# voutcn/megahit

Hardware: AMD Instinct MI355X
Metric: M (k+1)-mer edges sorted+counted/sec, sdbg_build k=21 (higher is better)
Workload: dtype u32; 1 GPU; read2sdbg (S1+S2) k=21 m=2 no mercy, 10000000 synthetic 150 bp PE reads per GPU (BASELINE configs[1]), inputs resident in HBM, outputs left in HBM; reads_per_gpu=10000000, edges_per_gpu=1290000000, k=21, min_count=2, parallelism=1 GPU, s1_items=1330000000, s2_items=117381042, sdbg_records=59857080

## Files before the change

### megahit_amd/csrc/mhx_internal.h

```cpp
#pragma once
#include <hip/hip_runtime.h>

#include <cstdint>
#include <cstdio>
#include <cstring>
#include <functional>
#include <map>
#include <stdexcept>
#include <string>
#include <vector>

#include "../../include/mhx.h"

namespace mhx {

struct OnesweepLaunch;
void set_error(const char *fmt, ...);

struct Error : std::runtime_error {
  explicit Error(const std::string &s) : std::runtime_error(s) {}
};

#define MHX_HIP(expr)                                                                          \
  do {                                                                                         \
// ... 99 lines not shown
    (ctx)->prof_begin(name, bytes);       \
    __VA_ARGS__;                          \
    MHX_HIP(hipGetLastError());           \
    (ctx)->prof_end();                    \
  } while (0)

namespace mhx {

struct SortPass {
  int shift;
  int bits;
  int shift2 = 0;
  int bits2 = 0;
  int prev_lo = -1;
};
struct SortPrep {
  const void *buf = nullptr;
  uint64_t n = 0;
  int hist_passes = 0;
  uint64_t hist_sig = 0;
  std::function<void(const OnesweepLaunch &)> gen;
  uint64_t gen_slots = 0;
  bool gen_var = false;
};
uint32_t *radix_sort(mhx_ctx *c, uint32_t *buf_a, uint32_t *buf_b, uint64_t n, int stride, int key_words,
                     const std::vector<SortPass> &passes, SortPrep *prep = nullptr);
uint32_t *sort_whole_key(mhx_ctx *c, uint32_t *buf_a, uint32_t *buf_b, uint64_t n, int stride, int key_words,
                         const std::vector<SortPass> &passes, SortPrep *prep = nullptr);
std::vector<SortPass> make_passes(int key_words, int lo_bit, int hi_bit);
bool sort_takes_generated_first_pass(const mhx_ctx *c, uint64_t n, int stride, const std::vector<SortPass> &passes);
uint64_t passes_signature(const std::vector<SortPass> &ps);
uint32_t *kmsort_exact(mhx_ctx *c, uint32_t *buf_a, uint32_t *buf_b, uint64_t n, int S, int key_words, SortPrep *prep = nullptr);

void exclusive_scan_u32_u64(mhx_ctx *c, const uint32_t *in, uint64_t *out, uint64_t n, uint64_t *d_total);
void exclusive_scan_u64(mhx_ctx *c, const uint64_t *in, uint64_t *out, uint64_t n, uint64_t *d_total);
void find_group_heads(mhx_ctx *c, const uint32_t *items, uint64_t n, int stride, int cmp_bits,
                      uint64_t *heads, uint64_t *d_count);
uint64_t count_group_heads(mhx_ctx *c, const uint32_t *items, uint64_t n, int stride, int cmp_bits);

struct DigitSpec;
DigitSpec spec_of_pass(const SortPass &ps, int key_words);
std::vector<SortPass> make_passes_ranges(int key_words, const std::vector<std::pair<int, int>> &ranges);
void emit_sdbg(mhx_ctx *c, const uint32_t *sorted, uint64_t n_items, int S, int kw, uint32_t k, int is_seq, mhx_sdbg_result *out, int compact_bits = 0);

void partition_by_owner(mhx_ctx *c, const uint32_t *a, uint32_t *b, uint64_t n, int stride, const uint8_t *lut, int n_parts,
                        uint64_t *counts);
uint64_t s1_extract(mhx_ctx *c, uint32_t k, bool compact, SortPrep *prep, bool defer_items = false, bool filter_in_gen = false);
bool s1_compact(const mhx_ctx *c, uint32_t k, int want_mercy);
bool s1_rank_tagged(const mhx_ctx *c, uint32_t k);
int s1_stride(uint32_t k, bool compact);
struct S1Sources {
  int n = 0;
  std::vector<const uint32_t *> ptr;
// ... 136 lines not shown
```

### megahit_amd/csrc/s1_skm.hip

```cpp
#include <cstring>

#include "s1_shared.h"

namespace mhx {

constexpr int kSkmC = 8;
constexpr int kSkmW = 10;
constexpr int kSkmNM = kSkmC + kSkmW - 1;
constexpr int kSkmMinBinBits = 16, kSkmMaxBinBits = 20;

__device__ __forceinline__ uint32_t skm_mix(uint32_t c) {
  uint32_t h = c * 0x9E3779B1u;
  return h ^ (h >> 15);
}
__device__ __forceinline__ uint32_t skm_mix2(uint32_t c) {
  uint32_t h = c * 0x9E3779B1u;
  h ^= h >> 15;
  return h * 0x85EBCA6Bu;
}
__device__ __forceinline__ uint32_t skm_bin_of(uint32_t minh) {
  return (minh ^ (minh >> 16)) * 0x7FEB352Du;
}

template <int NT, int J, bool VAR, bool COUNT = false>
__global__ __launch_bounds__(NT) void k_skm_make(const uint32_t *__restrict__ seq, const uint64_t *__restrict__ start, uint32_t L, uint32_t bpr, uint64_t n_blocks,
                                                 int k, int bin_bits, uint32_t bin_lo, uint32_t bin_hi, int count_items, uint64_t pos_base,
                                                 unsigned long long *__restrict__ hp, uint4 *__restrict__ out, unsigned long long cap,
                                                 unsigned long long *__restrict__ cursor, uint32_t *__restrict__ err, unsigned long long *__restrict__ digit_hist) {
  __shared__ uint32_t sm_scan[NT / kWave + 1];
  __shared__ unsigned long long s_base;
  __shared__ uint32_t dh[3][256];
  __shared__ uint32_t lbin[J * kSkmC][NT];
  __shared__ uint32_t hpl[2][12];
  const int tid = threadIdx.x;
  if (tid < 24) hpl[tid / 12][tid % 12] = 0;
  for (int i = tid; i < 768; i += NT) dh[i >> 8][i & 255] = 0;
  __syncthreads();
  const bool third_digit = bin_bits > 16;
  const int M = k + 1 - (kSkmW - 1);
  const uint32_t mmask = (1u << (2 * M)) - 1u;
  const int K1 = k + 1;
  const unsigned bin_sh = 32u - (unsigned)bin_bits;
  unsigned long long items = 0;
  uint32_t hp_n[2] = {0, 0};
  unsigned long long hp_p[2] = {~0ull, ~0ull};
  for (uint64_t it = blockIdx.x; it * (uint64_t)(NT * J) < n_blocks; it += gridDim.x) {
    uint64_t Wv[J], pos0[J];
    uint32_t smask[J], emask[J];
    uint32_t bflag[J];
#pragma unroll
    for (int j = 0; j < J; ++j) {
      const uint64_t b = it * (uint64_t)(NT * J) + (uint64_t)j * NT + tid;
      smask[j] = 0;
      emask[j] = 0;
      bflag[j] = 0;
      Wv[j] = 0;
      pos0[j] = 0;
      if (b < n_blocks) {
        const uint64_t r = b / bpr;
        const uint32_t q0 = (uint32_t)(b - r * bpr) * kSkmC;
        uint64_t base;
        uint32_t nwin;
        if constexpr (VAR) {
          base = start[r];
          const uint64_t len_r = start[r + 1] - base;
          nwin = len_r >= (uint64_t)K1 ? (uint32_t)(len_r - k) : 0u;
          if (q0 == 0 && nwin && count_items) items += nwin + (COUNT ? 0 : 4);
        } else {
          base = r * L;
          nwin = L - k;
        }
        if (q0 < nwin) {
// ... 2 lines not shown
          const unsigned sh = (unsigned)(a & 15) * 2;
          const uint32_t c0 = seq[wi], c1 = seq[wi + 1], c2 = seq[wi + 2];
          const uint64_t W = ((uint64_t)funnel_l(c0, c1, sh) << 32) | funnel_l(c1, c2, sh);
          const uint64_t R = rc64(W, 32);
          uint32_t h[kSkmNM];
#pragma unroll
          for (int i = 0; i < kSkmNM; ++i) {
            const uint32_t f = (uint32_t)(W >> (64 - 2 * (i + M))) & mmask;
            const uint32_t rv = (uint32_t)(R >> (2 * i)) & mmask;
            h[i] = skm_mix(min(f, rv));
          }
          uint32_t sfx[kSkmW];
          sfx[kSkmW - 1] = h[kSkmW - 1];
#pragma unroll
          for (int i = kSkmW - 2; i >= 0; --i) sfx[i] = min(h[i], sfx[i + 1]);
          uint32_t pfx = 0xFFFFFFFFu;
          uint32_t bins[kSkmC];
          bins[0] = skm_bin_of(sfx[0]) >> bin_sh;
#pragma unroll
          for (int w = 1; w < kSkmC; ++w) {
            pfx = min(pfx, h[kSkmW - 1 + w]);
            bins[w] = skm_bin_of(min(sfx[w], pfx)) >> bin_sh;
          }
#pragma unroll
          for (int w = 0; w < kSkmC; ++w) lbin[j * kSkmC + w][tid] = bins[w];
          const uint32_t n_here = min((uint32_t)kSkmC, nwin - q0);
          uint32_t km = 0, sm = 0, hm = 0;
          if (hp) {
            const uint64_t dx = W ^ (W << 2);
#pragma unroll
            for (int w = 0; w < kSkmC; ++w)
              if ((uint32_t)w < n_here && ((dx << (2 * w)) >> (64 - 2 * (K1 - 1))) == 0) hm |= 1u << w;
            if (hm && count_items) {
#pragma unroll
              for (int w = 0; w < kSkmC; ++w)
                if ((hm >> w) & 1u) {
                  const unsigned b = (unsigned)(W >> (62 - 2 * w)) & 3u;
                  const unsigned cls = b == 0 || b == 3 ? 0u : 1u;
                  if constexpr (COUNT) {
                    const bool strand = b >= 2;
                    const unsigned prev_raw = q0 + w == 0 ? kSentinel
                                              : (w == 0 ? (unsigned)((seq[(a - 1) >> 4] >> (30 - 2 * (unsigned)((a - 1) & 15))) & 3u) : (unsigned)(W >> (64 - 2 * w)) & 3u);
                    const unsigned next_raw = q0 + w + 1 == nwin ? kSentinel : (unsigned)(W >> (62 - 2 * (w + K1))) & 3u;
                    const unsigned pv = strand ? comp_or_sentinel(next_raw) : prev_raw, nx = strand ? comp_or_sentinel(prev_raw) : next_raw;
                    atomicAdd(&hpl[cls][0], 1u);
                    if (pv < 4) atomicAdd(&hpl[cls][1 + pv], 1u);
                    if (nx < 4) atomicAdd(&hpl[cls][5 + nx], 1u);
                  } else {
// ... 2 lines not shown
                  }
                }
            }
          }
#pragma unroll
          for (int w = 0; w < kSkmC; ++w)
            if ((uint32_t)w < n_here && !((hm >> w) & 1u) && bins[w] >= bin_lo && bins[w] < bin_hi) km |= 1u << w;
#pragma unroll
          for (int w = 0; w < kSkmC; ++w)
            if (((km >> w) & 1u) && (w == 0 || !((km >> (w - 1)) & 1u) || bins[w] != bins[w > 0 ? w - 1 : 0])) sm |= 1u << w;
          smask[j] = sm;
          emask[j] = km & ((sm >> 1) | ~(km >> 1));
          if constexpr (COUNT) {
            const uint64_t pb = a > 0 ? (uint64_t)((seq[(a - 1) >> 4] >> (30 - 2 * (unsigned)((a - 1) & 15))) & 3u) : 0ull;
            Wv[j] = (W >> 2) | (pb << 62);
            bflag[j] = (q0 == 0 ? 1u : 0u) | (q0 + n_here == nwin ? 2u : 0u) | (n_here << 2);
          } else {
            Wv[j] = W;
          }
          pos0[j] = pos_base + a;
        }
      }
    }
    uint32_t cnt = 0;
#pragma unroll
    for (int j = 0; j < J; ++j) cnt += (uint32_t)__builtin_popcount(smask[j]);
    uint32_t total = 0;
    const uint32_t excl = block_exclusive_sum<uint32_t, NT>(cnt, sm_scan, &total);
    if (tid == 0) s_base = total ? atomicAdd(cursor, (unsigned long long)total) : 0ull;
    __syncthreads();
    const unsigned long long base = s_base;
    if (base + total > cap) {
      if (tid == 0) atomicOr(err, 1u);
      return;
    }
    unsigned long long at = base + excl;
#pragma unroll
    for (int j = 0; j < J; ++j) {
      uint32_t sm = smask[j], em = emask[j];
      while (sm) {
        const int rs = __builtin_ctz(sm), re = __builtin_ctz(em);
        sm &= sm - 1;
        em &= em - 1;
        const int len = re - rs + 1;
        const uint32_t run_bin = lbin[j * kSkmC + rs][tid];
        const uint64_t p = pos0[j] + (uint64_t)rs;
        if constexpr (COUNT) {
          const uint64_t bases = (Wv[j] << (2 * rs)) & (~0ull << (64 - 2 * (K1 + len + 1)));
          const uint32_t n_blk = bflag[j] >> 2;
          const uint32_t fl = ((bflag[j] & 1u) && rs == 0 ? 16u : 0u) | ((bflag[j] & 2u) && (uint32_t)(re + 1) == n_blk ? 8u : 0u);
          out[at++] = make_uint4((run_bin << 8) | ((uint32_t)(p >> 32) << 28) | ((uint32_t)(len - 1) << 5) | fl, (uint32_t)(bases >> 32), (uint32_t)bases, (uint32_t)p);
        } else {
        const uint64_t bases = ((Wv[j] << (2 * rs)) & (~0ull << (64 - 2 * (K1 + len - 1)))) | (uint64_t)(len - 1);
        out[at++] = make_uint4((run_bin << 8) | ((uint32_t)(p >> 32) << 28), (uint32_t)(bases >> 32), (uint32_t)bases, (uint32_t)p);
        }
        atomicAdd(&dh[0][run_bin & 255u], 1u);
        atomicAdd(&dh[1][(run_bin >> 8) & 255u], 1u);
        if (third_digit) atomicAdd(&dh[2][run_bin >> 16], 1u);
      }
    }
  }
  if constexpr (VAR) {
    items = wave_sum(items);
    if ((tid & (kWave - 1)) == 0 && items) atomicAdd(cursor + 3, items);
  }
  if constexpr (COUNT) {
    __syncthreads();
    if (hp && count_items && tid < 24 && hpl[tid / 12][tid % 12]) atomicAdd(hp + 8 + (tid / 12) * 16 + (tid % 12), (unsigned long long)hpl[tid / 12][tid % 12]);
  }
  if (!COUNT && hp && count_items) {
#pragma unroll
    for (int x = 0; x < 2; ++x) {
      const uint32_t n_w = wave_sum(hp_n[x]);
      if (n_w) {
        unsigned long long pmin = hp_p[x];
#pragma unroll
        for (int d = kWave / 2; d > 0; d >>= 1) pmin = min(pmin, (unsigned long long)__shfl_xor((long long)pmin, d, kWave));
        if ((tid & (kWave - 1)) == 0) {
          atomicAdd(hp + x, (unsigned long long)n_w);
          atomicMin(hp + 2 + x, pmin);
        }
      }
    }
// ... 30 lines not shown
}

__global__ __launch_bounds__(256) void k_skm_bounds(const uint4 *__restrict__ recs, uint64_t n, uint32_t n_bins, uint64_t *__restrict__ bounds,
                                                    uint32_t *__restrict__ max_bin) {
  const uint32_t b = blockIdx.x * 256 + threadIdx.x;
  if (b > n_bins) return;
  auto lower = [&](uint32_t v) -> uint64_t {
    uint64_t lo = 0, hi = n;
    while (lo < hi) {
      const uint64_t mid = (lo + hi) >> 1;
      const uint32_t bin = (reinterpret_cast<const uint32_t *>(recs + mid)[0] >> 8) & 0xFFFFFu;
      if (bin < v) lo = mid + 1;
      else hi = mid;
    }
    return lo;
  };
  const uint64_t at = b == n_bins ? n : lower(b);
  bounds[b] = at;
  if (b < n_bins) {
    const uint64_t nx = b + 1 == n_bins ? n : lower(b + 1);
    const uint64_t d = nx - at;
    atomicMax(max_bin, d > 0xFFFFFFFFull ? 0xFFFFFFFFu : (uint32_t)d);
  }
}

struct SkmArgs {
  int k;
  uint32_t m;
  uint8_t *solid_bytes;
  unsigned long long *hist;
  uint2 *agg_raw;
  uint32_t agg_cap;
  uint32_t *agg_counts;
  uint32_t *err;
  uint32_t max_fill;
  int probe_limit;
  uint32_t bin_lo, bin_hi;
  unsigned long long *marks_raw;
  uint32_t marks_cap;
  uint32_t *marks_counts;
};
struct SkmSrcs {
  const uint4 *ptr[kSkmSrcMax];
  const uint64_t *bounds[kSkmSrcMax];
  int n;
};
// ... 862 lines not shown
  const double need = (double)n_win * (double)std::max<long long>(c->opt("s1_skm_cap_pct", 36), 1) / 100.0 * 32.0;
  const double budget = (double)std::max<long long>(c->opt("s1_skm_pass_gb", 48), 1) * 1e9;
  return (int)std::min(64.0, std::max(1.0, std::ceil(need / budget)));
}

bool s1_skm_front(mhx_ctx *c, uint32_t k, SkmFront *f, int pass, int n_passes, int bin_bits_agreed, bool for_count) {
  SeqSet &s = c->seqs;
  hipStream_t st = c->stream;
  const bool var = s.fixed_len == 0;
  const uint32_t L = var ? s.max_len : s.fixed_len, bpr = (L - k + kSkmC - 1) / kSkmC;
  const uint64_t n_blocks = s.n_seqs * (uint64_t)bpr;
  const uint64_t n_win = var ? (s.n_bases > s.n_seqs * (uint64_t)k ? s.n_bases - s.n_seqs * (uint64_t)k : 0) : s.n_seqs * (uint64_t)(L - k);
  const uint64_t cap_all = n_win * (uint64_t)std::max<long long>(c->opt("s1_skm_cap_pct", 36), 1) / 100;
  const uint64_t cap = std::max<uint64_t>(n_passes > 1 ? cap_all / n_passes + cap_all / n_passes * 15 / 100 : cap_all, 1u << 16);
  int bin_bits = kSkmMinBinBits;
  while (bin_bits < kSkmMaxBinBits && (double)n_win * 0.29 / (double)(1ull << bin_bits) > 8192.0) ++bin_bits;
  if (const long long fb = c->opt("s1_skm_bin_bits", 0)) bin_bits = (int)std::min<long long>(kSkmMaxBinBits, std::max<long long>(8, fb));
  if (bin_bits_agreed > 0) bin_bits = bin_bits_agreed;
  uint4 *buf_a = c->ws("items_a", cap * 16 + 64).as<uint4>();
  uint4 *buf_b = c->ws("items_b", cap * 16 + 64).as<uint4>();
  unsigned long long *cursor = c->ws("skm_cursor", 64).as<unsigned long long>();
  uint32_t *err = reinterpret_cast<uint32_t *>(cursor + 1);
  uint32_t *max_bin = err + 1;
  MHX_HIP(hipMemsetAsync(cursor, 0, 64, st));
  std::vector<SortPass> passes;
  for (int lo = 0; lo < bin_bits; lo += 8) passes.push_back(SortPass{8 + lo, std::min(8, bin_bits - lo), 0, 0, 0});
  unsigned long long *pre_hist = c->ws("sort_pre_hist", (size_t)kMaxFusedPasses * 256 * 8).as<unsigned long long>();
  MHX_HIP(hipMemsetAsync(pre_hist, 0, (size_t)3 * 256 * 8, st));
  constexpr int NT = 512, J = 2;
  const uint64_t cus = c->n_cus > 0 ? (uint64_t)c->n_cus : 256;
  const unsigned grid = (unsigned)std::min<uint64_t>(div_ceil(n_blocks, (uint64_t)NT * J), cus * 8);
  const uint32_t n_bins = 1u << bin_bits;
  const uint32_t bin_lo = (uint32_t)((uint64_t)n_bins * pass / n_passes), bin_hi = (uint32_t)((uint64_t)n_bins * (pass + 1) / n_passes);
  unsigned long long *hp = nullptr;
  if (!c->global_bases && c->opt("s1_skm_hp", 1)) {
    hp = c->ws("skm_hp", 512).as<unsigned long long>();
    if (pass == 0) {
      unsigned long long init[48] = {0};
      init[2] = init[3] = ~0ull;
      MHX_HIP(hipMemcpyAsync(hp, init, sizeof init, hipMemcpyHostToDevice, st));
      MHX_HIP(hipStreamSynchronize(st));
    }
  }
#define MHX_MAKE(VARV, COUNTV)                                                                                                                                   \
  hipLaunchKernelGGL((k_skm_make<NT, J, VARV, COUNTV>), dim3(grid), dim3(NT), 0, st, s.words.as<uint32_t>(), s.start.as<uint64_t>(), L, bpr, n_blocks, (int)k, \
                     bin_bits, bin_lo, bin_hi, pass == 0 ? 1 : 0, c->pos_base, hp, buf_a, (unsigned long long)cap, cursor, err, pre_hist)
  MHX_LAUNCH(c, for_count ? "count_skm_make" : "s1_skm_make", (double)s.n_bases / 4 + (double)n_win * 16 / 3.5, {
    if (var && for_count) MHX_MAKE(true, true);
    else if (var) MHX_MAKE(true, false);
    else if (for_count) MHX_MAKE(false, true);
    else MHX_MAKE(false, false);
  });
#undef MHX_MAKE
  unsigned long long h[4] = {0, 0, 0, 0};
  std::vector<unsigned long long> h_dh(passes.size() * 256);
  MHX_HIP(hipMemcpyAsync(h, cursor, 32, hipMemcpyDeviceToHost, st));
  MHX_HIP(hipMemcpyAsync(h_dh.data(), pre_hist, h_dh.size() * 8, hipMemcpyDeviceToHost, st));
  MHX_HIP(hipStreamSynchronize(st));
  f->n_records = 0;
  f->hp = hp;
  if ((uint32_t)h[1] != 0 || h[0] > cap) return false;
  const uint64_t n = h[0];
  {
    const uint64_t n_bins_pass = std::max<uint64_t>(1, ((1ull << bin_bits) + n_passes - 1) / n_passes);
    const uint64_t limit = std::max<uint64_t>((uint64_t)c->opt("s1_skm_max_bin", 1 << 16), 16 * (n / n_bins_pass + 1));
    bool all = n > 0;
    uint64_t smallest_excess = ~0ull;
    for (size_t p = 0; p < passes.size() && all; ++p) {
      const uint64_t vals = 1ull << passes[p].bits;
      uint64_t mx = 0;
      for (uint64_t d = 0; d < vals; ++d) mx = std::max<uint64_t>(mx, h_dh[p * 256 + d]);
      const uint64_t mean = n / std::max<uint64_t>(1, (p + 1 == passes.size() && n_passes > 1) ? std::max<uint64_t>(1, vals / n_passes) : vals);
      const uint64_t excess = mx > mean ? mx - mean : 0;
      smallest_excess = std::min(smallest_excess, excess);
      all = excess >= limit + limit / 2;
    }
    if (all) {
      f->n_records = n;
      f->max_bin = (uint32_t)std::min<uint64_t>(smallest_excess, 0xFFFFFFFFu);
      return false;
    }
  }
  SortPrep prep;
  prep.buf = buf_a;
  prep.n = n;
  prep.hist_passes = (int)passes.size();
  prep.hist_sig = passes_signature(passes);
  uint32_t *sorted = radix_sort(c, reinterpret_cast<uint32_t *>(buf_a), reinterpret_cast<uint32_t *>(buf_b), n, 4, 1, passes, &prep);
  uint64_t *bounds = c->ws("s1_bucket_bounds", ((size_t)n_bins + 1) * 8 + 64).as<uint64_t>();
  MHX_LAUNCH(c, "s1_skm_bounds", (double)n_bins * 8 * 30,
             hipLaunchKernelGGL(k_skm_bounds, dim3((n_bins + 1 + 255) / 256), dim3(256), 0, st, reinterpret_cast<const uint4 *>(sorted), n, n_bins, bounds, max_bin));
  uint32_t h_max = 0;
  MHX_HIP(hipMemcpyAsync(&h_max, max_bin, 4, hipMemcpyDeviceToHost, st));
  MHX_HIP(hipStreamSynchronize(st));
  f->n_src = 1;
  f->src[0] = reinterpret_cast<const uint4 *>(sorted);
  f->src_bounds[0] = bounds;
  f->spare = sorted == reinterpret_cast<uint32_t *>(buf_a) ? reinterpret_cast<uint32_t *>(buf_b) : reinterpret_cast<uint32_t *>(buf_a);
  f->spare_bytes = cap * 16;
  f->n_records = n;
  f->n_windows = n_win;
  if (pass == 0) f->n_items = var ? h[3] : s.n_seqs * (uint64_t)(L - k + (for_count ? 0 : 4));
  f->n_bins = n_bins;
  f->bin_lo = bin_lo;
  f->bin_hi = bin_hi;
  f->bin_bits = bin_bits;
  f->max_bin = h_max;
  const uint64_t limit = std::max<uint64_t>((uint64_t)c->opt("s1_skm_max_bin", 1 << 16), 16 * (n / (bin_hi - bin_lo) + 1));
  return h_max <= limit;
}

// ... 125 lines not shown
```

### megahit_amd/csrc/sort.hip

```cpp
#include "dev_prims.h"
#include <cstdlib>
#include <cstring>
#include <string>

#include "mhx_internal.h"
#include "sort_digits.h"
#include "sort_kernels.h"

namespace mhx {

template <int S, int NI>
__global__ __launch_bounds__(kSortThreads) void k_radix_hist(const uint32_t *__restrict__ items, uint64_t n, DigitSpec ds,
                                                             uint32_t *__restrict__ hist, uint64_t n_chunks,
                                                             const uint8_t *__restrict__ lut) {
  __shared__ uint32_t h[kSortWaves][256];
  for (int i = threadIdx.x; i < kSortWaves * 256; i += kSortThreads) (&h[0][0])[i] = 0;
  __syncthreads();
  const int w = threadIdx.x / kWave;
  const uint64_t base = (uint64_t)blockIdx.x * SortCfg<S, NI>::kChunk;
  for (int j = 0; j < SortCfg<S, NI>::kChunk / kSortThreads; ++j) {
    uint64_t idx = base + (uint64_t)j * kSortThreads + threadIdx.x;
    if (idx < n) {
      const uint32_t *p = items + idx * S;
      unsigned d;
// ... 202 lines not shown
    ds.wi2 = key_words - 1 - ps.shift2 / 32;
    ds.bit2 = (unsigned)(ps.shift2 % 32);
    ds.mask2 = (1u << ps.bits2) - 1;
    ds.sh2 = (unsigned)ps.bits;
  }
  if (ps.prev_lo >= 0 && ps.prev_lo < ps.shift && !ps.bits2 && ps.prev_lo / 32 == (ps.shift + ps.bits - 1) / 32) {
    const unsigned hi = (unsigned)(ps.shift % 32), lo = (unsigned)(ps.prev_lo % 32);
    ds.prev_mask = ((1u << hi) - 1u) & ~((1u << lo) - 1u);
  }
  return ds;
}

struct SortEnv {
  bool classic;
  std::string shape;
  int items;
};
static SortEnv sort_env() {
  const char *e = getenv("MHX_SORT"), *sh = getenv("MHX_SORT_SHAPE"), *it = getenv("MHX_SORT_ITEMS");
  return SortEnv{e && !strcmp(e, "classic"), sh ? sh : "", it ? atoi(it) : 0};
}
static void refuse_unconsumed_generator(const SortPrep &prep, const char *who) {
  if (prep.gen) throw Error(std::string(who) + ": the records of this buffer are to be made by a generated first pass, which this sort path cannot run");
}

template <int S, int NI, int UT>
static uint32_t *radix_sort_onesweep(mhx_ctx *c, uint32_t *a, uint32_t *b, uint64_t n, int key_words, const std::vector<SortPass> &passes,
                                     const SortPrep &prep) {
  const int P = (int)passes.size();
  const bool prep_fits = prep.buf == (const void *)a && prep.n == n;
  const bool gen = prep.gen && prep_fits && S == 3 && NI == 8 && UT == 3;
  if (!gen) refuse_unconsumed_generator(prep, "radix sort (chained scan)");
  const uint64_t gen_slots = gen ? std::max<uint64_t>(prep.gen_slots, n) : n;
  const int xcd_units = c->opt("sort_xcd_units", 1) != 0 && c->n_cus >= 192;
  const uint64_t unit = (uint64_t)kSortThreads * NI * UT;
  auto units_of = [&](uint64_t items) { return xcd_units ? (div_ceil(items, unit) + 127) / 128 * 128 : div_ceil(items, unit); };
  const uint64_t n_units = units_of(n), n_units_gen = units_of(gen_slots);
  hipStream_t st = c->stream;
  constexpr bool kCanUt2 = S == 3 && NI == 8 && UT == 3;
  const bool loaded_ut2 = kCanUt2 && c->opt("sort_loaded_ut2", 0) != 0;
  const uint64_t unit2 = (uint64_t)kSortThreads * NI * 2;
  const uint64_t n_units2 = xcd_units ? (div_ceil(n, unit2) + 127) / 128 * 128 : div_ceil(n, unit2);
  const uint64_t n_status = std::max(n_units_gen, loaded_ut2 ? n_units2 : 0);
  unsigned long long *status = c->ws("sort_status", n_status * 256 * 8).as<unsigned long long>();
  unsigned long long *gh = c->ws("sort_ghist", (size_t)2 * kMaxChainedPasses * 256 * 8).as<unsigned long long>();
  unsigned long long *starts = gh + kMaxChainedPasses * 256;
  constexpr int kErrSlot = kMaxChainedPasses * 8;
  uint32_t *tickets = c->ws("sort_tickets", (kErrSlot + 8) * 4).as<uint32_t>();
  MHX_HIP(hipMemsetAsync(status, 0, n_status * 256 * 8, st));
  MHX_HIP(hipMemsetAsync(gh, 0, (size_t)kMaxChainedPasses * 256 * 8, st));
  MHX_HIP(hipMemsetAsync(tickets, 0, (kErrSlot + 8) * 4, st));
  const double bytes = (double)n * S * 4;
  static const std::string nm_hist = "radix_hist_all_" + std::to_string(S * 4) + "B", nm_scat = "radix_scatter_" + std::to_string(S * 4) + "B";
  const unsigned hgrid = (unsigned)std::min<uint64_t>(div_ceil(n, (uint64_t)kSortThreads * 16), 4096);
  std::vector<DigitSpec> all(P);
  for (int p = 0; p < P; ++p) all[p] = spec_of_pass(passes[p], key_words);
  const bool pre = prep_fits && prep.hist_passes == P && P > 0 && P <= kMaxFusedPasses && prep.hist_sig == passes_signature(passes);
  if (gen && !pre) throw Error("radix sort: a generated first pass needs the digit histograms of the plan (pre-hist)");
  if (pre) MHX_HIP(hipMemcpyAsync(gh, c->work["sort_pre_hist"].p, (size_t)P * 256 * 8, hipMemcpyDeviceToDevice, st));
  for (int p0 = 0; p0 < P && !pre; p0 += kMaxFusedPasses) {
    DigitSpecs specs;
    specs.n = std::min(kMaxFusedPasses, P - p0);
    for (int p = 0; p < specs.n; ++p) specs.d[p] = all[p0 + p];
    MHX_LAUNCH(c, nm_hist.c_str(), bytes,
               hipLaunchKernelGGL((k_radix_hist_all<S>), dim3(hgrid), dim3(kSortThreads), 0, st, a, n, specs, gh + (size_t)p0 * 256));
  }
  hipLaunchKernelGGL(k_bin_starts, dim3(P), dim3(256), 0, st, gh, starts);
  constexpr bool kHasUnitRuns = (S <= 3 && NI == 8 && (UT == 3 || UT == 2)) || (S == 4 && NI == 8 && UT == 2) || (S > 4 && NI == 4 && UT == 2);
  const bool unit_runs = kHasUnitRuns && c->opt("sort_unit_runs", 1) != 0;
  const bool rank_uniform = unit_runs && c->opt("sort_rank_uniform", 1) != 0;
  for (int p = 0; p < P; ++p) {
    const int nb = passes[p].bits + passes[p].bits2;
    const int wi = digit_word_of(all[p], nb, 1);
    if (p == 0 && gen) {
      static const std::string nm_gen = nm_scat + "_gen";
      MHX_LAUNCH(c, nm_gen.c_str(), bytes,
                 prep.gen(OnesweepLaunch{(unsigned)n_units_gen, st, b, gen_slots, all[p], nb, starts + p * 256, status, tickets + p * 8,
                                    tickets + kErrSlot, (unsigned long long)(p + 1), xcd_units, unit_runs ? 1 : 0, wi}));
    } else if (unit_runs) {
      if constexpr (kHasUnitRuns) {
#define MHX_U(RANKV, WIV)                                                                                                                      \
  hipLaunchKernelGGL((k_radix_onesweep_u<S, NI, UT, SrcArray<S>, RANKV, WIV>), dim3((unsigned)n_units), dim3(kSortThreads), 0, st, SrcArray<S>{a}, b, \
                     n, all[p], nb, starts + p * 256, status, tickets + p * 8, tickets + kErrSlot, (unsigned long long)(p + 1), xcd_units)
#define MHX_U2(RANKV, WIV)                                                                                                                     \
  hipLaunchKernelGGL((k_radix_onesweep_u<S, NI, 2, SrcArray<S>, RANKV, WIV>), dim3((unsigned)n_units2), dim3(kSortThreads), 0, st, SrcArray<S>{a}, b, \
                     n, all[p], nb, starts + p * 256, status, tickets + p * 8, tickets + kErrSlot, (unsigned long long)(p + 1), xcd_units)
        if constexpr (kCanUt2) {
          if (loaded_ut2 && wi == 0) {
            MHX_LAUNCH(c, nm_scat.c_str(), 2 * bytes, {
              if (rank_uniform && all[p].prev_mask) MHX_U2(2, 0);
              else MHX_U2(0, 0);
            });
            std::swap(a, b);
            continue;
          }
        }
// ... 254 lines not shown
    case 3: return partition_impl<3>(c, a, b, n, lut, n_parts, counts);
    case 4: return partition_impl<4>(c, a, b, n, lut, n_parts, counts);
    case 6: return partition_impl<6>(c, a, b, n, lut, n_parts, counts);
    case 8: return partition_impl<8>(c, a, b, n, lut, n_parts, counts);
    case 10: return partition_impl<10>(c, a, b, n, lut, n_parts, counts);
    case 12: return partition_impl<12>(c, a, b, n, lut, n_parts, counts);
    case 14: return partition_impl<14>(c, a, b, n, lut, n_parts, counts);
    case 16: return partition_impl<16>(c, a, b, n, lut, n_parts, counts);
    case 18: return partition_impl<18>(c, a, b, n, lut, n_parts, counts);
    case 20: return partition_impl<20>(c, a, b, n, lut, n_parts, counts);
    default: throw Error("partition_by_owner: unsupported record stride");
  }
}

bool sort_takes_generated_first_pass(const mhx_ctx *c, uint64_t n, int stride, const std::vector<SortPass> &passes) {
  (void)c;
  const SortEnv env = sort_env();
  if (env.classic) return false;
  if ((!env.shape.empty() && env.shape != "8x3") || (env.items && env.items != default_items<3>())) return false;
  return stride == 3 && n > 0 && passes.size() <= (size_t)kMaxChainedPasses && passes.size() <= (size_t)kMaxFusedPasses &&
         div_ceil(n, (uint64_t)kSortThreads * 8) < (1ull << 31);
}

uint32_t *radix_sort(mhx_ctx *c, uint32_t *a, uint32_t *b, uint64_t n, int stride, int key_words,
                     const std::vector<SortPass> &passes, SortPrep *prep_io) {
  SortPrep prep;
  if (prep_io) std::swap(prep, *prep_io);
  switch (stride) {
    case 2: return radix_sort_impl<2>(c, a, b, n, key_words, passes, prep);
    case 3: return radix_sort_impl<3>(c, a, b, n, key_words, passes, prep);
    case 4: return radix_sort_impl<4>(c, a, b, n, key_words, passes, prep);
    case 6: return radix_sort_impl<6>(c, a, b, n, key_words, passes, prep);
    case 8: return radix_sort_impl<8>(c, a, b, n, key_words, passes, prep);
    case 10: return radix_sort_impl<10>(c, a, b, n, key_words, passes, prep);
    case 12: return radix_sort_impl<12>(c, a, b, n, key_words, passes, prep);
    case 14: return radix_sort_impl<14>(c, a, b, n, key_words, passes, prep);
    case 16: return radix_sort_impl<16>(c, a, b, n, key_words, passes, prep);
    case 18: return radix_sort_impl<18>(c, a, b, n, key_words, passes, prep);
    case 20: return radix_sort_impl<20>(c, a, b, n, key_words, passes, prep);
    default: throw Error("radix_sort: unsupported record stride");
  }
}

}
```

### megahit_amd/csrc/sort_kernels.h

```cpp
#pragma once
#include "dev_prims.h"
#include "sort_digits.h"

namespace mhx {

constexpr int kSortThreads = 256;
constexpr int kSortWaves = kSortThreads / kWave;

template <int S>
constexpr int default_items() {
  return (S <= 4) ? 4 : (S <= 8 ? 8 : (S <= 12 ? 5 : (S <= 16 ? 4 : 3)));
}
template <int S, int ITEMS>
struct SortCfg {
  static constexpr int kItems = ITEMS;
  static constexpr int kTile = kSortThreads * kItems;
  static constexpr int kTilesPerChunk = (16384 / kTile) > 4 ? (16384 / kTile) : 4;
  static constexpr int kChunk = kTile * kTilesPerChunk;
};

template <int S>
struct Rec {
  uint32_t w[S];
};
// ... 47 lines not shown
__device__ __forceinline__ unsigned rec_digit2(const Rec<S> &r, const DigitSpec &ds) {
  unsigned d = rec_digit<S>(r, ds.wi1, ds.bit1, ds.mask1);
  if (ds.mask2) d |= rec_digit<S>(r, ds.wi2, ds.bit2, ds.mask2) << ds.sh2;
  return d;
}
__device__ __forceinline__ unsigned mem_digit(const uint32_t *p, int wi, unsigned bit, unsigned mask) {
  uint64_t v = p[wi];
  if (bit + (32 - __builtin_clz(mask)) > 32 && wi > 0) v |= (uint64_t)p[wi - 1] << 32;
  return (unsigned)(v >> bit) & mask;
}


template <int S>
struct SrcArray {
  const uint32_t *in;
  static constexpr bool kMayDrop = false;
  __device__ __forceinline__ bool is_record(const Rec<S> &) const { return true; }
  template <int NI>
  __device__ __forceinline__ void get(uint64_t first, uint64_t n, Rec<S> (&rec)[NI]) const {
#pragma unroll
    for (int j = 0; j < NI; ++j) {
      const uint64_t gi = first + (uint64_t)j * kWave;
      if (gi < n) load_rec<S>(in + gi * S, rec[j]);
    }
  }
  template <int NI>
  __device__ __forceinline__ uint64_t index(uint64_t tile_base, int w, int lane, int j) const {
    return tile_base + (uint64_t)(w * (kWave * NI) + j * kWave + lane);
  }
  template <int NI, int UT>
  __device__ __forceinline__ void get_unit(uint64_t unit_base, int w, int lane, uint64_t n, Rec<S> (&rec)[UT][NI]) const {
#pragma unroll
    for (int t = 0; t < UT; ++t) get<NI>(unit_base + (uint64_t)t * (kSortThreads * NI) + (uint64_t)(w * (kWave * NI) + lane), n, rec[t]);
  }
};

constexpr unsigned long long kStValMask = (1ull << 56) - 1;

template <int S, int NI, int UT, class Src, bool ANY_ORDER = false>
__global__ __launch_bounds__(kSortThreads) void k_radix_onesweep(Src src, uint32_t *__restrict__ out, uint64_t n,
                                                                 DigitSpec ds, int nbits, const unsigned long long *__restrict__ bin_start,
                                                                 unsigned long long *__restrict__ status, uint32_t *__restrict__ ticket,
                                                                 uint32_t *__restrict__ err, unsigned long long tag, int xcd_units) {
  constexpr int kTile = kSortThreads * NI;
  __shared__ __attribute__((aligned(16))) uint32_t stage[kTile * S];
  __shared__ uint32_t wave_cnt[kSortWaves][256];
// ... 324 lines not shown
```

Before: 52320 M edges/s.

## Scatter super-k-mer records into low-digit ranges during generation to skip first sort pass

The super-k-mer generation kernel gains a SPLIT mode. Each block stages records in shared memory per low bin digit and flushes them in 16-record groups into 256 fixed-capacity ranges through per-range atomic cursors, so the output already counts as partitioned by the first radix digit. The radix sort then skips that pass, reading the ranged layout through a new SrcRanged source that uses a prefix-sum kernel over the digit histogram. The aim is to remove one full read/write sort pass. In exchange it adds shared-memory staging, extra barriers, a smaller grid and a fallback re-run of the generator when any range overflows.

Result: slower. 37870 M edges/s (-27.6%).

```diff
diff --git a/megahit_amd/csrc/mhx_internal.h b/megahit_amd/csrc/mhx_internal.h
--- a/megahit_amd/csrc/mhx_internal.h
+++ b/megahit_amd/csrc/mhx_internal.h
@@ -145,6 +145,9 @@
   std::function<void(const OnesweepLaunch &)> gen;
   uint64_t gen_slots = 0;
   bool gen_var = false;
+  const unsigned long long *ranged_pfx = nullptr;
+  uint64_t range_cap = 0;
+  int hist_skip = 0;
 };
 uint32_t *radix_sort(mhx_ctx *c, uint32_t *buf_a, uint32_t *buf_b, uint64_t n, int stride, int key_words,
                      const std::vector<SortPass> &passes, SortPrep *prep = nullptr);
@@ -152,6 +155,7 @@
                          const std::vector<SortPass> &passes, SortPrep *prep = nullptr);
 std::vector<SortPass> make_passes(int key_words, int lo_bit, int hi_bit);
 bool sort_takes_generated_first_pass(const mhx_ctx *c, uint64_t n, int stride, const std::vector<SortPass> &passes);
+bool sort_takes_ranged_first_pass(const mhx_ctx *c, int stride, const std::vector<SortPass> &passes);
 uint64_t passes_signature(const std::vector<SortPass> &ps);
 uint32_t *kmsort_exact(mhx_ctx *c, uint32_t *buf_a, uint32_t *buf_b, uint64_t n, int S, int key_words, SortPrep *prep = nullptr);
 
diff --git a/megahit_amd/csrc/s1_skm.hip b/megahit_amd/csrc/s1_skm.hip
--- a/megahit_amd/csrc/s1_skm.hip
+++ b/megahit_amd/csrc/s1_skm.hip
@@ -22,18 +22,57 @@
   return (minh ^ (minh >> 16)) * 0x7FEB352Du;
 }
 
-template <int NT, int J, bool VAR, bool COUNT = false>
+constexpr int kSkmStage = 16;
+template <int NT>
+__device__ __forceinline__ void skm_flush(const uint4 (*stage)[kSkmStage], uint32_t *fill, uint32_t *__restrict__ rcur, uint32_t rcap,
+                                          uint4 *__restrict__ out, uint32_t *__restrict__ err, int tid, uint32_t min_fill) {
+  static_assert(kSkmStage == 16 && NT % 16 == 0 && (256 * 16) % NT == 0, "16 lanes per range");
+  constexpr int kIt = 256 * kSkmStage / NT;
+  const int s = tid & 15, g = tid >> 4, leader = (tid & (kWave - 1)) & ~15;
+  uint32_t cnt[kIt], base[kIt];
+#pragma unroll
+  for (int q = 0; q < kIt; ++q) {
+    const int d = q * (NT / 16) + g;
+    uint32_t n_out = 0, b = 0;
+    if (s == 0) {
+      const uint32_t f = fill[d];
+      if (f >= min_fill) {
+        n_out = min(f, (uint32_t)kSkmStage);
+        b = atomicAdd(&rcur[d], n_out);
+        fill[d] = 0;
+      }
+    }
+    cnt[q] = n_out;
+    base[q] = b;
+  }
+#pragma unroll
+  for (int q = 0; q < kIt; ++q) {
+    const int d = q * (NT / 16) + g;
+    const uint32_t n_out = __shfl(cnt[q], leader, kWave), b = __shfl(base[q], leader, kWave);
+    if ((uint32_t)s < n_out) {
+      if ((uint64_t)b + n_out <= (uint64_t)rcap) out[(uint64_t)d * rcap + b + (uint32_t)s] = stage[d][s];
+      else if (s == 0) atomicOr(err, 2u);
+    }
+  }
+}
+
+template <int NT, int J, bool VAR, bool COUNT = false, bool SPLIT = false>
 __global__ __launch_bounds__(NT) void k_skm_make(const uint32_t *__restrict__ seq, const uint64_t *__restrict__ start, uint32_t L, uint32_t bpr, uint64_t n_blocks,
                                                  int k, int bin_bits, uint32_t bin_lo, uint32_t bin_hi, int count_items, uint64_t pos_base,
                                                  unsigned long long *__restrict__ hp, uint4 *__restrict__ out, unsigned long long cap,
-                                                 unsigned long long *__restrict__ cursor, uint32_t *__restrict__ err, unsigned long long *__restrict__ digit_hist) {
+                                                 unsigned long long *__restrict__ cursor, uint32_t *__restrict__ err, unsigned long long *__restrict__ digit_hist,
+                                                 uint32_t *__restrict__ rcur, uint32_t rcap) {
   __shared__ uint32_t sm_scan[NT / kWave + 1];
   __shared__ unsigned long long s_base;
   __shared__ uint32_t dh[3][256];
-  __shared__ uint32_t lbin[J * kSkmC][NT];
+  __shared__ uint32_t lbin[SPLIT ? 1 : J * kSkmC][NT];
+  __shared__ __attribute__((aligned(16))) uint4 stage[SPLIT ? 256 : 1][kSkmStage];
+  __shared__ uint32_t fill[SPLIT ? 256 : 1];
   __shared__ uint32_t hpl[2][12];
   const int tid = threadIdx.x;
   if (tid < 24) hpl[tid / 12][tid % 12] = 0;
+  if constexpr (SPLIT)
+    for (int i = tid; i < 256; i += NT) fill[i] = 0;
   for (int i = tid; i < 768; i += NT) dh[i >> 8][i & 255] = 0;
   __syncthreads();
   const bool third_digit = bin_bits > 16;
@@ -48,6 +87,7 @@
     uint64_t Wv[J], pos0[J];
     uint32_t smask[J], emask[J];
     uint32_t bflag[J];
+    uint32_t binr[SPLIT ? J : 1][kSkmC];
 #pragma unroll
     for (int j = 0; j < J; ++j) {
       const uint64_t b = it * (uint64_t)(NT * J) + (uint64_t)j * NT + tid;
@@ -96,8 +136,13 @@
             pfx = min(pfx, h[kSkmW - 1 + w]);
             bins[w] = skm_bin_of(min(sfx[w], pfx)) >> bin_sh;
           }
-#pragma unroll
-          for (int w = 0; w < kSkmC; ++w) lbin[j * kSkmC + w][tid] = bins[w];
+          if constexpr (SPLIT) {
+#pragma unroll
+            for (int w = 0; w < kSkmC; ++w) binr[j][w] = bins[w];
+          } else {
+#pragma unroll
+            for (int w = 0; w < kSkmC; ++w) lbin[j * kSkmC + w][tid] = bins[w];
+          }
           const uint32_t n_here = min((uint32_t)kSkmC, nwin - q0);
           uint32_t km = 0, sm = 0, hm = 0;
           if (hp) {
@@ -146,6 +191,56 @@
         }
       }
     }
+    auto record_of = [&](int j, int rs, int re, uint32_t run_bin) -> uint4 {
+      const int len = re - rs + 1;
+      const uint64_t p = pos0[j] + (uint64_t)rs;
+      if constexpr (COUNT) {
+        const uint64_t bases = (Wv[j] << (2 * rs)) & (~0ull << (64 - 2 * (K1 + len + 1)));
+        const uint32_t n_blk = bflag[j] >> 2;
+        const uint32_t fl = ((bflag[j] & 1u) && rs == 0 ? 16u : 0u) | ((bflag[j] & 2u) && (uint32_t)(re + 1) == n_blk ? 8u : 0u);
+        return make_uint4((run_bin << 8) | ((uint32_t)(p >> 32) << 28) | ((uint32_t)(len - 1) << 5) | fl, (uint32_t)(bases >> 32), (uint32_t)bases, (uint32_t)p);
+      } else {
+        const uint64_t bases = ((Wv[j] << (2 * rs)) & (~0ull << (64 - 2 * (K1 + len - 1)))) | (uint64_t)(len - 1);
+        return make_uint4((run_bin << 8) | ((uint32_t)(p >> 32) << 28), (uint32_t)(bases >> 32), (uint32_t)bases, (uint32_t)p);
+      }
+    };
+    if constexpr (SPLIT) {
+      for (int round = 0;; ++round) {
+        bool waits = false;
+#pragma unroll
+        for (int j = 0; j < J; ++j) {
+          uint32_t sm = smask[j], em = emask[j], wsm = 0, wem = 0;
+          while (sm) {
+            const int rs = __builtin_ctz(sm), re = __builtin_ctz(em);
+            const uint32_t sbit = sm & (0u - sm), ebit = em & (0u - em);
+            sm ^= sbit;
+            em ^= ebit;
+            uint32_t run_bin = binr[j][0];
+#pragma unroll
+            for (int w = 1; w < kSkmC; ++w) run_bin = rs == w ? binr[j][w] : run_bin;
+            const uint32_t d = run_bin & 255u;
+            const uint32_t slot = atomicAdd(&fill[d], 1u);
+            if (slot < (uint32_t)kSkmStage) {
+              stage[d][slot] = record_of(j, rs, re, run_bin);
+              atomicAdd(&dh[0][d], 1u);
+              atomicAdd(&dh[1][(run_bin >> 8) & 255u], 1u);
+              if (third_digit) atomicAdd(&dh[2][run_bin >> 16], 1u);
+            } else {
+              wsm |= sbit;
+              wem |= ebit;
+            }
+          }
+          smask[j] = wsm;
+          emask[j] = wem;
+          waits = waits || wsm != 0;
+        }
+        const int any_waits = __syncthreads_or(waits ? 1 : 0);
+        if (round > 0 && !any_waits) break;
+        skm_flush<NT>(stage, fill, rcur, rcap, out, err, tid, (uint32_t)kSkmStage);
+        __syncthreads();
+        if (!any_waits) break;
+      }
+    } else {
     uint32_t cnt = 0;
 #pragma unroll
     for (int j = 0; j < J; ++j) cnt += (uint32_t)__builtin_popcount(smask[j]);
@@ -166,23 +261,18 @@
         const int rs = __builtin_ctz(sm), re = __builtin_ctz(em);
         sm &= sm - 1;
         em &= em - 1;
-        const int len = re - rs + 1;
         const uint32_t run_bin = lbin[j * kSkmC + rs][tid];
-        const uint64_t p = pos0[j] + (uint64_t)rs;
-        if constexpr (COUNT) {
-          const uint64_t bases = (Wv[j] << (2 * rs)) & (~0ull << (64 - 2 * (K1 + len + 1)));
-          const uint32_t n_blk = bflag[j] >> 2;
-          const uint32_t fl = ((bflag[j] & 1u) && rs == 0 ? 16u : 0u) | ((bflag[j] & 2u) && (uint32_t)(re + 1) == n_blk ? 8u : 0u);
-          out[at++] = make_uint4((run_bin << 8) | ((uint32_t)(p >> 32) << 28) | ((uint32_t)(len - 1) << 5) | fl, (uint32_t)(bases >> 32), (uint32_t)bases, (uint32_t)p);
-        } else {
-        const uint64_t bases = ((Wv[j] << (2 * rs)) & (~0ull << (64 - 2 * (K1 + len - 1)))) | (uint64_t)(len - 1);
-        out[at++] = make_uint4((run_bin << 8) | ((uint32_t)(p >> 32) << 28), (uint32_t)(bases >> 32), (uint32_t)bases, (uint32_t)p);
-        }
+        out[at++] = record_of(j, rs, re, run_bin);
         atomicAdd(&dh[0][run_bin & 255u], 1u);
         atomicAdd(&dh[1][(run_bin >> 8) & 255u], 1u);
         if (third_digit) atomicAdd(&dh[2][run_bin >> 16], 1u);
       }
     }
+    }
+  }
+  if constexpr (SPLIT) {
+    __syncthreads();
+    skm_flush<NT>(stage, fill, rcur, rcap, out, err, tid, 1u);
   }
   if constexpr (VAR) {
     items = wave_sum(items);
@@ -259,6 +349,15 @@
     const uint64_t d = nx - at;
     atomicMax(max_bin, d > 0xFFFFFFFFull ? 0xFFFFFFFFu : (uint32_t)d);
   }
+}
+
+__global__ __launch_bounds__(256) void k_skm_range_pfx(const unsigned long long *__restrict__ low_hist, unsigned long long *__restrict__ pfx) {
+  __shared__ unsigned long long sm[256 / kWave + 1];
+  const unsigned long long v = low_hist[threadIdx.x];
+  unsigned long long total = 0;
+  const unsigned long long ex = block_exclusive_sum<unsigned long long, 256>(v, sm, &total);
+  pfx[threadIdx.x] = ex;
+  if (threadIdx.x == 255) pfx[256] = total;
 }
 
 struct SkmArgs {
@@ -1167,14 +1266,16 @@
   unsigned long long *cursor = c->ws("skm_cursor", 64).as<unsigned long long>();
   uint32_t *err = reinterpret_cast<uint32_t *>(cursor + 1);
   uint32_t *max_bin = err + 1;
-  MHX_HIP(hipMemsetAsync(cursor, 0, 64, st));
   std::vector<SortPass> passes;
   for (int lo = 0; lo < bin_bits; lo += 8) passes.push_back(SortPass{8 + lo, std::min(8, bin_bits - lo), 0, 0, 0});
   unsigned long long *pre_hist = c->ws("sort_pre_hist", (size_t)kMaxFusedPasses * 256 * 8).as<unsigned long long>();
-  MHX_HIP(hipMemsetAsync(pre_hist, 0, (size_t)3 * 256 * 8, st));
   constexpr int NT = 512, J = 2;
   const uint64_t cus = c->n_cus > 0 ? (uint64_t)c->n_cus : 256;
-  const unsigned grid = (unsigned)std::min<uint64_t>(div_ceil(n_blocks, (uint64_t)NT * J), cus * 8);
+  const std::vector<SortPass> passes_rest(passes.begin() + (passes.size() > 1 ? 1 : 0), passes.end());
+  const uint32_t rcap = (uint32_t)std::min<uint64_t>(cap / 256 / kSkmStage * kSkmStage, 0xFFFFFF00u);
+  bool split = passes.size() > 1 && rcap > 0 && c->opt("s1_skm_split", 1) != 0 && sort_takes_ranged_first_pass(c, 4, passes_rest);
+  uint32_t *rcur = c->ws("skm_range_cursor", 257 * 8 + 256 * 4).as<uint32_t>() + 257 * 2;
+  unsigned long long *range_pfx = c->ws("skm_range_cursor", 257 * 8 + 256 * 4).as<unsigned long long>();
   const uint32_t n_bins = 1u << bin_bits;
   const uint32_t bin_lo = (uint32_t)((uint64_t)n_bins * pass / n_passes), bin_hi = (uint32_t)((uint64_t)n_bins * (pass + 1) / n_passes);
   unsigned long long *hp = nullptr;
@@ -1187,25 +1288,52 @@
       MHX_HIP(hipStreamSynchronize(st));
     }
   }
-#define MHX_MAKE(VARV, COUNTV)                                                                                                                                   \
-  hipLaunchKernelGGL((k_skm_make<NT, J, VARV, COUNTV>), dim3(grid), dim3(NT), 0, st, s.words.as<uint32_t>(), s.start.as<uint64_t>(), L, bpr, n_blocks, (int)k, \
-                     bin_bits, bin_lo, bin_hi, pass == 0 ? 1 : 0, c->pos_base, hp, buf_a, (unsigned long long)cap, cursor, err, pre_hist)
-  MHX_LAUNCH(c, for_count ? "count_skm_make" : "s1_skm_make", (double)s.n_bases / 4 + (double)n_win * 16 / 3.5, {
-    if (var && for_count) MHX_MAKE(true, true);
-    else if (var) MHX_MAKE(true, false);
-    else if (for_count) MHX_MAKE(false, true);
-    else MHX_MAKE(false, false);
-  });
-#undef MHX_MAKE
   unsigned long long h[4] = {0, 0, 0, 0};
   std::vector<unsigned long long> h_dh(passes.size() * 256);
-  MHX_HIP(hipMemcpyAsync(h, cursor, 32, hipMemcpyDeviceToHost, st));
-  MHX_HIP(hipMemcpyAsync(h_dh.data(), pre_hist, h_dh.size() * 8, hipMemcpyDeviceToHost, st));
-  MHX_HIP(hipStreamSynchronize(st));
+  auto make = [&](bool splitv) {
+    const unsigned grid = (unsigned)std::min<uint64_t>(div_ceil(n_blocks, (uint64_t)NT * J), cus * (splitv ? 2 : 8));
+    MHX_HIP(hipMemsetAsync(cursor, 0, 64, st));
+    MHX_HIP(hipMemsetAsync(pre_hist, 0, (size_t)3 * 256 * 8, st));
+    if (splitv) MHX_HIP(hipMemsetAsync(rcur, 0, 256 * 4, st));
+#define MHX_MAKE(VARV, COUNTV)                                                                                                                  \
+  do {                                                                                                                                         \
+    if (splitv)                                                                                                                                \
+      hipLaunchKernelGGL((k_skm_make<NT, J, VARV, COUNTV, true>), dim3(grid), dim3(NT), 0, st, s.words.as<uint32_t>(), s.start.as<uint64_t>(), L, bpr, \
+                         n_blocks, (int)k, bin_bits, bin_lo, bin_hi, pass == 0 ? 1 : 0, c->pos_base, hp, buf_a, (unsigned long long)cap, cursor, err, \
+                         pre_hist, rcur, rcap);                                                                                                \
+    else                                                                                                                                       \
+      hipLaunchKernelGGL((k_skm_make<NT, J, VARV, COUNTV, false>), dim3(grid), dim3(NT), 0, st, s.words.as<uint32_t>(), s.start.as<uint64_t>(), L, bpr, \
+                         n_blocks, (int)k, bin_bits, bin_lo, bin_hi, pass == 0 ? 1 : 0, c->pos_base, hp, buf_a, (unsigned long long)cap, cursor, err, \
+                         pre_hist, rcur, rcap);                                                                                                \
+  } while (0)
+    MHX_LAUNCH(c, for_count ? "count_skm_make" : "s1_skm_make", (double)s.n_bases / 4 + (double)n_win * 16 / 3.5, {
+      if (var && for_count) MHX_MAKE(true, true);
+      else if (var) MHX_MAKE(true, false);
+      else if (for_count) MHX_MAKE(false, true);
+      else MHX_MAKE(false, false);
+    });
+#undef MHX_MAKE
+    if (splitv) hipLaunchKernelGGL(k_skm_range_pfx, dim3(1), dim3(256), 0, st, pre_hist, range_pfx);
+    MHX_HIP(hipMemcpyAsync(h, cursor, 32, hipMemcpyDeviceToHost, st));
+    MHX_HIP(hipMemcpyAsync(h_dh.data(), pre_hist, h_dh.size() * 8, hipMemcpyDeviceToHost, st));
+    MHX_HIP(hipStreamSynchronize(st));
+  };
+  make(split);
   f->n_records = 0;
   f->hp = hp;
-  if ((uint32_t)h[1] != 0 || h[0] > cap) return false;
-  const uint64_t n = h[0];
+  auto records_made = [&]() {
+    if (!split) return (uint64_t)h[0];
+    uint64_t sum = 0;
+    for (int d = 0; d < 256; ++d) sum += h_dh[d];
+    return sum;
+  };
+  bool range_overflow = false;
+  if (split) {
+    range_overflow = ((uint32_t)h[1] & 2u) != 0;
+    for (int d = 0; d < 256; ++d) range_overflow = range_overflow || h_dh[d] > rcap;
+  }
+  if (((uint32_t)h[1] & ~2u) != 0 || (!split && h[0] > cap)) return false;
+  uint64_t n = records_made();
   {
     const uint64_t n_bins_pass = std::max<uint64_t>(1, ((1ull << bin_bits) + n_passes - 1) / n_passes);
     const uint64_t limit = std::max<uint64_t>((uint64_t)c->opt("s1_skm_max_bin", 1 << 16), 16 * (n / n_bins_pass + 1));
@@ -1226,12 +1354,30 @@
       return false;
     }
   }
+  if (range_overflow) {
+    if (hp && pass == 0) {
+      unsigned long long init[48] = {0};
+      init[2] = init[3] = ~0ull;
+      MHX_HIP(hipMemcpyAsync(hp, init, sizeof init, hipMemcpyHostToDevice, st));
+      MHX_HIP(hipStreamSynchronize(st));
+    }
+    split = false;
+    make(false);
+    if ((uint32_t)h[1] != 0 || h[0] > cap) return false;
+    n = h[0];
+  }
   SortPrep prep;
   prep.buf = buf_a;
   prep.n = n;
-  prep.hist_passes = (int)passes.size();
-  prep.hist_sig = passes_signature(passes);
-  uint32_t *sorted = radix_sort(c, reinterpret_cast<uint32_t *>(buf_a), reinterpret_cast<uint32_t *>(buf_b), n, 4, 1, passes, &prep);
+  const std::vector<SortPass> &sort_passes = split ? passes_rest : passes;
+  prep.hist_passes = (int)sort_passes.size();
+  prep.hist_sig = passes_signature(sort_passes);
+  if (split) {
+    prep.ranged_pfx = range_pfx;
+    prep.range_cap = rcap;
+    prep.hist_skip = 1;
+  }
+  uint32_t *sorted = radix_sort(c, reinterpret_cast<uint32_t *>(buf_a), reinterpret_cast<uint32_t *>(buf_b), n, 4, 1, sort_passes, &prep);
   uint64_t *bounds = c->ws("s1_bucket_bounds", ((size_t)n_bins + 1) * 8 + 64).as<uint64_t>();
   MHX_LAUNCH(c, "s1_skm_bounds", (double)n_bins * 8 * 30,
              hipLaunchKernelGGL(k_skm_bounds, dim3((n_bins + 1 + 255) / 256), dim3(256), 0, st, reinterpret_cast<const uint4 *>(sorted), n, n_bins, bounds, max_bin));
diff --git a/megahit_amd/csrc/sort.hip b/megahit_amd/csrc/sort.hip
--- a/megahit_amd/csrc/sort.hip
+++ b/megahit_amd/csrc/sort.hip
@@ -248,6 +248,7 @@
 }
 static void refuse_unconsumed_generator(const SortPrep &prep, const char *who) {
   if (prep.gen) throw Error(std::string(who) + ": the records of this buffer are to be made by a generated first pass, which this sort path cannot run");
+  if (prep.ranged_pfx) throw Error(std::string(who) + ": the records of this buffer lie in ranges, which this sort path cannot read");
 }
 
 template <int S, int NI, int UT>
@@ -256,7 +257,9 @@
   const int P = (int)passes.size();
   const bool prep_fits = prep.buf == (const void *)a && prep.n == n;
   const bool gen = prep.gen && prep_fits && S == 3 && NI == 8 && UT == 3;
-  if (!gen) refuse_unconsumed_generator(prep, "radix sort (chained scan)");
+  constexpr bool kCanRanged = S == 4 && NI == 8 && UT == 2;
+  const bool ranged = kCanRanged && prep.ranged_pfx && prep_fits && !prep.gen;
+  if (!gen && !ranged) refuse_unconsumed_generator(prep, "radix sort (chained scan)");
   const uint64_t gen_slots = gen ? std::max<uint64_t>(prep.gen_slots, n) : n;
   const int xcd_units = c->opt("sort_xcd_units", 1) != 0 && c->n_cus >= 192;
   const uint64_t unit = (uint64_t)kSortThreads * NI * UT;
@@ -281,9 +284,12 @@
   const unsigned hgrid = (unsigned)std::min<uint64_t>(div_ceil(n, (uint64_t)kSortThreads * 16), 4096);
   std::vector<DigitSpec> all(P);
   for (int p = 0; p < P; ++p) all[p] = spec_of_pass(passes[p], key_words);
-  const bool pre = prep_fits && prep.hist_passes == P && P > 0 && P <= kMaxFusedPasses && prep.hist_sig == passes_signature(passes);
+  const bool pre = prep_fits && prep.hist_passes == P && P > 0 && P + prep.hist_skip <= kMaxFusedPasses && prep.hist_sig == passes_signature(passes);
   if (gen && !pre) throw Error("radix sort: a generated first pass needs the digit histograms of the plan (pre-hist)");
-  if (pre) MHX_HIP(hipMemcpyAsync(gh, c->work["sort_pre_hist"].p, (size_t)P * 256 * 8, hipMemcpyDeviceToDevice, st));
+  if (ranged && !pre) throw Error("radix sort: records in ranges need the digit histograms of the plan (pre-hist)");
+  if (pre)
+    MHX_HIP(hipMemcpyAsync(gh, static_cast<const unsigned long long *>(c->work["sort_pre_hist"].p) + (size_t)prep.hist_skip * 256, (size_t)P * 256 * 8,
+                           hipMemcpyDeviceToDevice, st));
   for (int p0 = 0; p0 < P && !pre; p0 += kMaxFusedPasses) {
     DigitSpecs specs;
     specs.n = std::min(kMaxFusedPasses, P - p0);
@@ -295,9 +301,26 @@
   constexpr bool kHasUnitRuns = (S <= 3 && NI == 8 && (UT == 3 || UT == 2)) || (S == 4 && NI == 8 && UT == 2) || (S > 4 && NI == 4 && UT == 2);
   const bool unit_runs = kHasUnitRuns && c->opt("sort_unit_runs", 1) != 0;
   const bool rank_uniform = unit_runs && c->opt("sort_rank_uniform", 1) != 0;
+  if (ranged && (!unit_runs || digit_word_of(all[0], passes[0].bits + passes[0].bits2, 1) != 0))
+    throw Error("radix sort: records in ranges need the unit-wide pass on a digit of the first word");
   for (int p = 0; p < P; ++p) {
     const int nb = passes[p].bits + passes[p].bits2;
     const int wi = digit_word_of(all[p], nb, 1);
+    if constexpr (kCanRanged) {
+      if (p == 0 && ranged) {
+#define MHX_R(RANKV)                                                                                                                              \
+  hipLaunchKernelGGL((k_radix_onesweep_u<S, NI, UT, SrcRanged<S>, RANKV, 0>), dim3((unsigned)n_units), dim3(kSortThreads), 0, st,                  \
+                     SrcRanged<S>{a, prep.ranged_pfx, prep.range_cap}, b, n, all[p], nb, starts + p * 256, status, tickets + p * 8, tickets + kErrSlot, \
+                     (unsigned long long)(p + 1), xcd_units)
+        MHX_LAUNCH(c, nm_scat.c_str(), 2 * bytes, {
+          if (rank_uniform && all[p].prev_mask) MHX_R(2);
+          else MHX_R(0);
+        });
+#undef MHX_R
+        std::swap(a, b);
+        continue;
+      }
+    }
     if (p == 0 && gen) {
       static const std::string nm_gen = nm_scat + "_gen";
       MHX_LAUNCH(c, nm_gen.c_str(), bytes,
@@ -598,6 +621,14 @@
          div_ceil(n, (uint64_t)kSortThreads * 8) < (1ull << 31);
 }
 
+bool sort_takes_ranged_first_pass(const mhx_ctx *c, int stride, const std::vector<SortPass> &passes) {
+  const SortEnv env = sort_env();
+  if (env.classic || (!env.shape.empty() && env.shape != "8x2") || (env.items && env.items != default_items<4>())) return false;
+  if (stride != 4 || passes.empty() || passes.size() > (size_t)kMaxChainedPasses || passes.size() + 1 > (size_t)kMaxFusedPasses) return false;
+  if (c->opt("sort_unit_runs", 1) == 0) return false;
+  return digit_word_of(spec_of_pass(passes[0], 1), passes[0].bits + passes[0].bits2, 1) == 0;
+}
+
 uint32_t *radix_sort(mhx_ctx *c, uint32_t *a, uint32_t *b, uint64_t n, int stride, int key_words,
                      const std::vector<SortPass> &passes, SortPrep *prep_io) {
   SortPrep prep;
diff --git a/megahit_amd/csrc/sort_kernels.h b/megahit_amd/csrc/sort_kernels.h
--- a/megahit_amd/csrc/sort_kernels.h
+++ b/megahit_amd/csrc/sort_kernels.h
@@ -93,6 +93,52 @@
     for (int j = 0; j < NI; ++j) {
       const uint64_t gi = first + (uint64_t)j * kWave;
       if (gi < n) load_rec<S>(in + gi * S, rec[j]);
+    }
+  }
+  template <int NI>
+  __device__ __forceinline__ uint64_t index(uint64_t tile_base, int w, int lane, int j) const {
+    return tile_base + (uint64_t)(w * (kWave * NI) + j * kWave + lane);
+  }
+  template <int NI, int UT>
+  __device__ __forceinline__ void get_unit(uint64_t unit_base, int w, int lane, uint64_t n, Rec<S> (&rec)[UT][NI]) const {
+#pragma unroll
+    for (int t = 0; t < UT; ++t) get<NI>(unit_base + (uint64_t)t * (kSortThreads * NI) + (uint64_t)(w * (kWave * NI) + lane), n, rec[t]);
+  }
+};
+template <int S>
+struct SrcRanged {
+  const uint32_t *in;
+  const unsigned long long *pfx;
+  uint64_t range_cap;
+  static constexpr bool kMayDrop = false;
+  __device__ __forceinline__ bool is_record(const Rec<S> &) const { return true; }
+  __device__ __forceinline__ int range_of(uint64_t gi, uint64_t n) const {
+    int d = (int)((gi << 8) / n);
+    if (pfx[d] <= gi && gi < pfx[d + 1]) return d;
+    int lo = 0, hi = 256;
+    while (hi - lo > 1) {
+      const int mid = (lo + hi) >> 1;
+      if (pfx[mid] <= gi) lo = mid;
+      else hi = mid;
+    }
+    return lo;
+  }
+  template <int NI>
+  __device__ __forceinline__ void get(uint64_t first, uint64_t n, Rec<S> (&rec)[NI]) const {
+    if (first >= n) return;
+    int d = range_of(first, n);
+    uint64_t lo = pfx[d], hi = pfx[d + 1];
+#pragma unroll
+    for (int j = 0; j < NI; ++j) {
+      const uint64_t gi = first + (uint64_t)j * kWave;
+      if (gi < n) {
+        while (gi >= hi) {
+          ++d;
+          lo = hi;
+          hi = pfx[d + 1];
+        }
+        load_rec<S>(in + ((uint64_t)d * range_cap + (gi - lo)) * S, rec[j]);
+      }
     }
   }
   template <int NI>
```
